# commanderson/morna

Measured on NVIDIA B200. Metric: exact kNN queries/s (50k samples x 3000 feats, k=100), higher is better.
Workload: dtype fp16 first pass (fp32 accumulate), f64 re-rank

## Files before the change

morna_b200/csrc/search_batched.cu:

```cuda
#include <cuda_fp16.h>
#include <limits.h>
#include <math.h>

#include "common.cuh"
#include "tc_ptx.cuh"

namespace morna {

constexpr int kPrepThreads = 256;

__global__ void __launch_bounds__(kPrepThreads)
prep_samples_kernel(const float *__restrict__ vectors, const double *__restrict__ pp, int64_t n, int64_t ld,
                    __half *__restrict__ hs, int64_t ld_h, float *__restrict__ rho_max) {
    const int lane = threadIdx.x & 31;
    const int64_t warps_total = (int64_t)gridDim.x * (kPrepThreads / 32);
    const int chunks = (int)(ld >> 2), chunks_h = (int)(ld_h >> 2);
    for (int64_t row = (int64_t)blockIdx.x * (kPrepThreads / 32) + (threadIdx.x >> 5); row < n; row += warps_total) {
        const float4 *src = reinterpret_cast<const float4 *>(vectors + row * ld);
        uint2 *dst = reinterpret_cast<uint2 *>(hs + row * ld_h);
        const double norm = sqrt(pp[row]);
        const double inv = norm > 0.0 ? 1.0 / norm : 0.0;
        double res = 0.0;
        for (int c = lane; c < chunks_h; c += 32) {
            float4 v = c < chunks ? ldg_stream_f4(src + c) : make_float4(0.f, 0.f, 0.f, 0.f);
// ... 637 lines not shown
                                if (j < valid) dst[j] = __uint_as_float(r[j]);
                        }
                    }
                } else {
                    uint32_t mask = 0;
#pragma unroll
                    for (int j = 0; j < 32; ++j)
                        mask |= (uint32_t)(__uint_as_float(r[j]) >= thr && j < valid) << j;
                    if (mask) {
                        int at = atomicAdd(p.cand_cnt + row, __popc(mask));
                        float *cs = p.cand_score + (int64_t)row * p.cap;
                        int32_t *ci = p.cand_id + (int64_t)row * p.cap;
#pragma unroll
                        for (int j = 0; j < 32; ++j) {
                            if ((mask >> j) & 1u) {
                                if (at < p.cap) { cs[at] = __uint_as_float(r[j]); ci[at] = p.id_base + col0 + j; }
                                ++at;
                            }
                        }
                    }
                }
            }
            tc_fence_before();
            mbar_arrive(tempty_bar(acc));
            if (++acc == ACC_STAGES) { acc = 0; acc_phase ^= 1; }
        }
    }
    tc_fence_before();
    __syncthreads();
    if (warp == 2) tmem_dealloc<1>(tmem_base, TMEM_COLS);
}

namespace gemm2 {
constexpr int BM = 128, BN = 256, BN_HALF = 128, BK = 64, UMMA_K = 16;
constexpr int A_BYTES = BM * BK * 2, B_BYTES = BN_HALF * BK * 2, STAGE_BYTES = A_BYTES + B_BYTES;
constexpr int THREADS = 192;
constexpr int HELPER_WARPS = 8;
constexpr int THREADS_ALL = THREADS + 32 * HELPER_WARPS;
constexpr int ACC_STAGES = 2, TMEM_COLS = ACC_STAGES * BN;
constexpr int HELPER_BYTES = HELPER_WARPS * 1024 * 4 + 16;
constexpr int smem_bytes(int stages) { return stages * STAGE_BYTES + 1024 + 256 + HELPER_BYTES; }
}

__device__ __forceinline__ uint32_t cluster_ctarank() {
    uint32_t r;
    asm volatile("mov.u32 %0, %%cluster_ctarank;" : "=r"(r));
    return r;
}
__device__ __forceinline__ void cluster_sync_all() {
    asm volatile("barrier.cluster.arrive.release.aligned;\n\tbarrier.cluster.wait.acquire.aligned;" ::: "memory");
}
__device__ __forceinline__ uint32_t mapa_rank(uint32_t addr, uint32_t rank) {
    uint32_t r;
    asm volatile("mapa.shared::cluster.u32 %0, %1, %2;" : "=r"(r) : "r"(addr), "r"(rank));
    return r;
}

template <int kStages, bool kHelpers, int kCluster>
__device__ __forceinline__ void
knn_gemm2_body(const CUtensorMap &tmap_q, const CUtensorMap &tmap_s, const GemmParams &p, const RerankParams &rr) {
    using namespace gemm2;
    constexpr bool kQuad = kCluster == 4;
    using namespace tc;
    extern __shared__ uint8_t smem_raw[];
    const uint32_t base = (smem_u32(smem_raw) + 1023u) & ~1023u;
    const uint32_t bars = base + kStages * STAGE_BYTES;
    auto full_bar = [&](int s) { return bars + 8u * s; };
    auto empty_bar = [&](int s) { return bars + 8u * (kStages + s); };
    auto tfull_bar = [&](int a) { return bars + 8u * (2 * kStages + a); };
    auto tempty_bar = [&](int a) { return bars + 8u * (2 * kStages + ACC_STAGES + a); };
    const uint32_t tmem_slot = bars + 8u * (2 * kStages + 2 * ACC_STAGES);
    volatile uint32_t *tmem_slot_ptr =
        reinterpret_cast<volatile uint32_t *>(smem_raw + (tmem_slot - smem_u32(smem_raw)));
    int *helper_lists = reinterpret_cast<int *>(smem_raw + (bars + 256u - smem_u32(smem_raw)));
    volatile int *helper_stop = helper_lists + (kHelpers ? HELPER_WARPS * 1024 : 0);

    const int warp = threadIdx.x >> 5, lane = threadIdx.x & 31;
    const uint32_t crank = cluster_ctarank();
    const uint32_t rank = crank & 1u;
    const uint32_t leader_rank = crank & ~1u;
    const int pair_in_cluster = (int)(crank >> 1);
    const bool leader = rank == 0;
    if (warp == 0 && lane == 0) {
        prefetch_tmap(&tmap_q);
        prefetch_tmap(&tmap_s);
    }
    if (warp == 1 && lane == 0) {
        for (int s = 0; s < kStages; ++s) { mbar_init(full_bar(s), 1); mbar_init(empty_bar(s), kQuad ? 2 : 1); }
        for (int a = 0; a < ACC_STAGES; ++a) { mbar_init(tfull_bar(a), 1); mbar_init(tempty_bar(a), 256); }
        fence_barrier_init();
        *helper_stop = 0;
    }
    if (warp == 2) {
        tmem_alloc<2>(tmem_slot, TMEM_COLS);
        tmem_relinquish<2>();
    }
    tc_fence_before();
    cluster_sync_all();
    tc_fence_after();
    const uint32_t tmem_base = *tmem_slot_ptr;

    const int pair = blockIdx.x / kCluster, pairs = gridDim.x / kCluster;
    const int m_pairs = (p.m_blocks + 1) >> 1;
    const int m_groups = kQuad ? (m_pairs + 1) >> 1 : m_pairs;
    const int total_tiles = m_groups * p.n_tiles;
    auto m_pair_of = [&](int t) { return kQuad ? 2 * (t % m_groups) + pair_in_cluster : t % m_groups; };
    if (warp == 0) {
        if (lane == 0) {
            int stage = 0; uint32_t phase = 0;
            uint64_t keep = 0;
            if (p.l2_keep) asm volatile("createpolicy.fractional.L2::evict_last.b64 %0, 1.0;" : "=l"(keep));
            for (int t = pair; t < total_tiles; t += pairs) {
                const int m_pair = m_pair_of(t), n_tile = t / m_groups;
                const int row_q = m_pair * 2 * BM + (int)rank * BM;
                const int row_s = p.n_begin + n_tile * BN + (int)rank * BN_HALF + (kQuad ? pair_in_cluster * (BN_HALF / 2) : 0);
                for (int kb = 0; kb < p.kblocks; ++kb) {
                    if (p.relaxed_ns > 1) mbar_wait_relaxed(empty_bar(stage), phase ^ 1, 20u);
                    else mbar_wait(empty_bar(stage), phase ^ 1);
                    const uint32_t a_dst = base + stage * STAGE_BYTES, b_dst = a_dst + A_BYTES;
                    const uint32_t bar0 = mapa_rank(full_bar(stage), leader_rank);
                    if (leader) mbar_expect_tx(full_bar(stage), 2 * STAGE_BYTES);
                    if (p.l2_keep) tma_load_2d_pair_hint(a_dst, &tmap_q, bar0, kb * BK, row_q, keep);
                    else tma_load_2d_pair(a_dst, &tmap_q, bar0, kb * BK, row_q);
                    if (kQuad)
                        tma_load_2d_pair_multicast(b_dst + pair_in_cluster * (B_BYTES / 2), &tmap_s, bar0, kb * BK, row_s,
                                                   (uint16_t)((1u << crank) | (1u << (crank ^ 2u))));
                    else if (p.l2_keep)
                        tma_load_2d_pair_hint(b_dst, &tmap_s, bar0, kb * BK, row_s, keep);
                    else
                        tma_load_2d_pair(b_dst, &tmap_s, bar0, kb * BK, row_s);
                    if (++stage == kStages) { stage = 0; phase ^= 1; }
                }
            }
        }
    } else if (warp == 1) {
        if (lane == 0 && leader) {
            constexpr uint32_t idesc = instr_desc_f16(2 * BM, BN,  0);
            int stage = 0; uint32_t phase = 0; int acc = 0; uint32_t acc_phase = 0;
            long long w_full = 0, w_acc = 0;
            const long long t_begin = clock64();
            for (int t = pair; t < total_tiles; t += pairs) {
                long long c0 = p.debug ? clock64() : 0;
                mbar_wait(tempty_bar(acc), acc_phase ^ 1);
                if (p.debug) w_acc += clock64() - c0;
                tc_fence_after();
                const uint32_t d_tmem = tmem_base + acc * BN;
                for (int kb = 0; kb < p.kblocks; ++kb) {
                    c0 = p.debug ? clock64() : 0;
                    mbar_wait(full_bar(stage), phase);
                    if (p.debug) w_full += clock64() - c0;
                    tc_fence_after();
                    const uint32_t a_src = base + stage * STAGE_BYTES, b_src = a_src + A_BYTES;
                    const uint64_t da = smem_desc_sw128(a_src), db = smem_desc_sw128(b_src);
#pragma unroll
                    for (int k = 0; k < BK / UMMA_K; ++k)
                        umma_f16<2>(d_tmem, da + 2 * k, db + 2 * k, idesc, (kb | k) != 0);
                    umma_commit_pair(empty_bar(stage), kQuad ? 0xF : 0x3);
                    if (kb == p.kblocks - 1) umma_commit_pair(tfull_bar(acc), (uint16_t)(0x3u << leader_rank));
                    if (++stage == kStages) { stage = 0; phase ^= 1; }
                }
                if (++acc == ACC_STAGES) { acc = 0; acc_phase ^= 1; }
            }
            if (p.debug) { p.debug[blockIdx.x * 4 + 0] = w_full; p.debug[blockIdx.x * 4 + 1] = w_acc; p.debug[blockIdx.x * 4 + 2] = clock64() - t_begin; }
        }
    } else if (kHelpers && warp >= THREADS / 32) {
        if (rr.queue) rerank_warp_loop<8, 2>(rr, helper_lists + (warp - THREADS / 32) * 1024, lane, helper_stop);
    } else {
        const int quarter = warp & 3;
        int acc = 0; uint32_t acc_phase = 0;
        long long e_busy = 0;
        for (int t = pair; t < total_tiles; t += pairs) {
            const int m_pair = m_pair_of(t), n_tile = t / m_groups;
            const int row = m_pair * 2 * BM + (int)rank * BM + quarter * 32 + lane;
            const bool row_ok = row < p.nq;
            const int col_tile = p.n_begin + n_tile * BN;
            float thr = INFINITY;
            if (p.mode == 1 && row_ok) thr = p.thr[row];
            if (p.relaxed_ns) mbar_wait_relaxed(tfull_bar(acc), acc_phase, (unsigned)p.relaxed_ns);
            else mbar_wait(tfull_bar(acc), acc_phase);
            const long long e0 = p.debug ? clock64() : 0;
            tc_fence_after();
            const uint32_t taddr = tmem_base + ((uint32_t)(quarter * 32) << 16) + acc * BN;
#pragma unroll 1
            for (int c = 0; c < BN / 32; ++c) {
                uint32_t r[32];
                tmem_ld_32x32(taddr + c * 32, r);
                tmem_ld_wait();
                const int col0 = col_tile + c * 32;
                const int valid = min(32, p.n_end - col0);
                if (p.mode == 0) {
                    if (row_ok && valid > 0) {
                        float *dst = p.pilot + (int64_t)row * p.pilot_ld + (col0 - p.n_begin);
                        if (valid == 32) {
#pragma unroll
                            for (int j = 0; j < 32; j += 4)
                                *reinterpret_cast<float4 *>(dst + j) =
                                    make_float4(__uint_as_float(r[j]), __uint_as_float(r[j + 1]),
                                                __uint_as_float(r[j + 2]), __uint_as_float(r[j + 3]));
                        } else {
#pragma unroll
                            for (int j = 0; j < 32; ++j)
                                if (j < valid) dst[j] = __uint_as_float(r[j]);
                        }
                    }
                } else {
                    uint32_t mask = 0;
#pragma unroll
                    for (int j = 0; j < 32; ++j)
                        mask |= (uint32_t)(__uint_as_float(r[j]) >= thr && j < valid) << j;
                    if (mask && !p.dry_epilogue) {
                        int at = atomicAdd(p.cand_cnt + row, __popc(mask));
                        float *cs = p.cand_score + (int64_t)row * p.cap;
                        int32_t *ci = p.cand_id + (int64_t)row * p.cap;
#pragma unroll
                        for (int j = 0; j < 32; ++j) {
                            if ((mask >> j) & 1u) {
                                if (at < p.cap) { cs[at] = __uint_as_float(r[j]); ci[at] = p.id_base + col0 + j; }
                                ++at;
                            }
                        }
                    }
                }
            }
            tc_fence_before();
            mbar_arrive_cluster(tempty_bar(acc), leader_rank);
            if (p.debug) e_busy += clock64() - e0;
            if (++acc == ACC_STAGES) { acc = 0; acc_phase ^= 1; }
        }
        if (p.debug && warp == 2 && lane == 0) p.debug[blockIdx.x * 4 + 3] = e_busy;
        if (warp == 2 && lane == 0) *helper_stop = 1;
    }
    tc_fence_before();
    cluster_sync_all();
    if (warp == 2) tmem_dealloc<2>(tmem_base, TMEM_COLS);
}

template <int kStages, bool kHelpers>
__global__ void __cluster_dims__(2, 1, 1) __launch_bounds__(kHelpers ? gemm2::THREADS_ALL : gemm2::THREADS, 1)
knn_gemm2_kernel(const __grid_constant__ CUtensorMap tmap_q, const __grid_constant__ CUtensorMap tmap_s, GemmParams p,
                 const RerankParams rr) {
    knn_gemm2_body<kStages, kHelpers, 2>(tmap_q, tmap_s, p, rr);
}

template <int kStages>
__global__ void __cluster_dims__(4, 1, 1) __launch_bounds__(gemm2::THREADS, 1)
knn_gemm4_kernel(const __grid_constant__ CUtensorMap tmap_q, const __grid_constant__ CUtensorMap tmap_s, GemmParams p,
                 const RerankParams rr) {
    knn_gemm2_body<kStages, false, 4>(tmap_q, tmap_s, p, rr);
}

constexpr int kKthThreads = 256, kKthItems = 32, kKthMax = kKthThreads * kKthItems;

__device__ __forceinline__ uint32_t float_key(float v) {
    uint32_t b = __float_as_uint(v);
    return (b & 0x80000000u) ? ~b : (b | 0x80000000u);
}
__device__ __forceinline__ float key_float(uint32_t k) {
    return __uint_as_float((k & 0x80000000u) ? (k & 0x7fffffffu) : ~k);
}

struct KthParams {
    int32_t k, n0, n_begin, id_base, cap, fcap;
    const float *pilot; int64_t pilot_ld;
    const float *eps;
    float *thr;
    float *cand_score; int32_t *cand_id; int32_t *cand_cnt;
    float *cand2_score; int32_t *cand2_id;
    int32_t *fin_id; int32_t *fin_cnt;
    uint8_t *overflow; int32_t *stats;
    float *kth_bound;
};

template <int kItems>
__device__ __forceinline__ uint32_t warp_kth_largest(const uint32_t (&key)[kItems], int kk) {
    uint32_t hi = 0u, lo = ~0u;
#pragma unroll
    for (int j = 0; j < kItems; ++j) { hi = max(hi, key[j]); lo = min(lo, key[j] ? key[j] : ~0u); }
    hi = __reduce_max_sync(kFull, hi);
    lo = __reduce_min_sync(kFull, lo);
    if (hi == 0u || kk <= 0) return 0u;
    const int first = 31 - __clz((int)(hi ^ lo) | 1);
// ... 283 lines not shown
    CUresult r = fn(map, CU_TENSOR_MAP_DATA_TYPE_FLOAT16, 2, const_cast<void *>(ptr), dims, strides, box, estr,
                    CU_TENSOR_MAP_INTERLEAVE_NONE, CU_TENSOR_MAP_SWIZZLE_128B, promo, CU_TENSOR_MAP_FLOAT_OOB_FILL_NONE);
    if (r != CUDA_SUCCESS) { g_last_cuda_error = (int)r; return MORNA_ERR_CUDA; }
    return MORNA_OK;
}

static int sm_count_b() { return sm_count_current(); }

constexpr int kCandCap = kCandCapConst, kFinCap = 1024, kPilotMax = kKthMax;
constexpr int64_t kBatchedMaxRows = (int64_t)1 << 24;

static int g_gemm_pair = 1;
static int g_gemm_stages = 4;
static int g_block_rows = 131072;
static int g_pilot_rows = kKthMax;
static int g_block_growth = 1;
static int g_first_block = 0;
static int g_rerank_ctas_per_sm = 0;
static int g_rerank_rows = 4;
static int g_rerank_phase_mb = -1;
static int g_rerank_kernel = 1;
static int g_rerank_ctas = 0;
static int g_rerank_subs = 0;
static int g_side_job = 0;
static int g_rerank_sort_rows = 1;
static int g_rerank_evict_first = 0;
static int g_gemm_l2_keep = 0;
static int g_rerank_fat_sms = 0;
static int g_gemm_pairs_cap = 0;
static int g_rerank_pipe = 1;
static long long *g_gemm_debug = nullptr;
static int g_gemm_relaxed_ns = 0;
static int g_gemm_dry = 0;
static int g_carveout_hint = 0;
static int g_rerank_oneshot = 1;


static int launch_knn_gemm(const CUtensorMap &tmap_q, const CUtensorMap &tmap_s, const GemmParams &gp, cudaStream_t s,
                           const RerankParams *side = nullptr) {
    if (!g_gemm_pair) {
        int rca = ensure_dynamic_smem((const void *)knn_gemm_kernel, gemm::SMEM_BYTES);
        if (rca != MORNA_OK) return rca;
        int tiles = gp.m_blocks * gp.n_tiles;
        int grid = tiles < sm_count_b() ? tiles : sm_count_b();
        knn_gemm_kernel<<<grid, gemm::THREADS, gemm::SMEM_BYTES, s>>>(tmap_q, tmap_s, gp);
        MORNA_LAUNCH_CHECK();
        return MORNA_OK;
    }
    if (g_gemm_pair == 2 && !side && (gp.m_blocks % 4) == 0) {
        auto kern4 = knn_gemm4_kernel<4>;
        const int smem4 = gemm2::smem_bytes(4) - gemm2::HELPER_BYTES + 16;
        int rca = ensure_dynamic_smem((const void *)kern4, smem4);
        if (rca != MORNA_OK) return rca;
        int tiles4 = (gp.m_blocks / 4) * gp.n_tiles;
        int clusters = 0;
        cudaLaunchConfig_t cfg{};
        cfg.gridDim = dim3(4 * (sm_count_b() / 4)); cfg.blockDim = dim3(gemm2::THREADS); cfg.dynamicSmemBytes = smem4; cfg.stream = s;
        if (cudaOccupancyMaxActiveClusters(&clusters, kern4, &cfg) != cudaSuccess || clusters < 1) { cudaGetLastError(); clusters = sm_count_b() / 4; }
        if (clusters > sm_count_b() / 4) clusters = sm_count_b() / 4;
        if (tiles4 < clusters) clusters = tiles4;
        RerankParams none{};
        kern4<<<4 * clusters, gemm2::THREADS, smem4, s>>>(tmap_q, tmap_s, gp, none);
        MORNA_LAUNCH_CHECK();
        return MORNA_OK;
    }
    const int stages = g_gemm_stages == 4 ? 4 : 6;
    auto kern = side ? (stages == 4 ? knn_gemm2_kernel<4, true> : knn_gemm2_kernel<6, true>)
                     : (stages == 4 ? knn_gemm2_kernel<4, false> : knn_gemm2_kernel<6, false>);
    const int smem = gemm2::smem_bytes(stages);
    int rca = ensure_dynamic_smem((const void *)kern, smem);
    if (rca != MORNA_OK) return rca;
    int tiles = ((gp.m_blocks + 1) / 2) * gp.n_tiles;
    int pairs = sm_count_b() / 2;
    if (g_gemm_pairs_cap > 0 && pairs > g_gemm_pairs_cap) pairs = g_gemm_pairs_cap;
    if (tiles < pairs) pairs = tiles;
    RerankParams rr{};
    if (side) rr = *side;
    if (g_carveout_hint) cudaFuncSetAttribute((const void *)kern, cudaFuncAttributePreferredSharedMemoryCarveout, cudaSharedmemCarveoutMaxShared);
    const int threads = side ? gemm2::THREADS_ALL : gemm2::THREADS;
    const int smem_launch = side ? smem : smem - gemm2::HELPER_BYTES + 16;
    kern<<<2 * pairs, threads, smem_launch, s>>>(tmap_q, tmap_s, gp, rr);
    MORNA_LAUNCH_CHECK();
    return MORNA_OK;
}

struct BatchWs {
    size_t hq, qq, eps, pilot, thr, cand_score, cand_id, cand2_score, cand2_id, cand_cnt, fin_id, fin_cnt, fin_dist, queue, total;
    int64_t nq_pad, n0, pilot_ld;
};
static BatchWs batch_ws_layout(int64_t n, int64_t nq, int64_t ld_h) {
    BatchWs w{};
    w.nq_pad = (nq + 2 * gemm::BM - 1) / (2 * gemm::BM) * (2 * gemm::BM);
    w.n0 = n < g_pilot_rows ? n : g_pilot_rows;
    if (w.n0 > g_block_rows) w.n0 = g_block_rows;
    w.pilot_ld = (w.n0 + 3) / 4 * 4;
    size_t off = 0;
    auto take = [&](size_t bytes) { size_t at = off; off += align_up(bytes, 256); return at; };
    w.hq = take((size_t)w.nq_pad * ld_h * sizeof(__half));
    w.qq = take((size_t)nq * sizeof(double));
    w.eps = take((size_t)nq * sizeof(float));
    w.pilot = take((size_t)nq * w.pilot_ld * sizeof(float));
    w.thr = take((size_t)nq * sizeof(float));
    w.cand_score = take((size_t)nq * kCandCap * sizeof(float));
    w.cand_id = take((size_t)nq * kCandCap * sizeof(int32_t));
    if (n > g_block_rows || (g_first_block > 0 && n > g_first_block)) {
        w.cand2_score = take((size_t)nq * kCandCap * sizeof(float));
        w.cand2_id = take((size_t)nq * kCandCap * sizeof(int32_t));
    }
    w.cand_cnt = take((size_t)nq * sizeof(int32_t));
    w.fin_id = take((size_t)nq * kFinCap * sizeof(int32_t));
    w.fin_cnt = take((size_t)nq * sizeof(int32_t));
    w.fin_dist = take((size_t)nq * kFinCap * sizeof(double));
    w.queue = take(sizeof(unsigned long long));
    w.total = off + 1024;
// ... 53 lines not shown
        if (rcj != MORNA_OK) return rcj;
        if (warp_kernel && side_jobs_enabled()) side_ptr = &side;
    }
    cudaStream_t s = (cudaStream_t)stream;
    unsigned char *ws = (unsigned char *)workspace;
    __half *hq = (__half *)(ws + w.hq);
    double *qq = (double *)(ws + w.qq);
    float *eps = (float *)(ws + w.eps);
    float *pilot = (float *)(ws + w.pilot);
    float *thr = (float *)(ws + w.thr);
    float *cand_score = (float *)(ws + w.cand_score);
    int32_t *cand_id = (int32_t *)(ws + w.cand_id);
    int32_t *cand_cnt = (int32_t *)(ws + w.cand_cnt);
    int32_t *fin_id = (int32_t *)(ws + w.fin_id);
    int32_t *fin_cnt = (int32_t *)(ws + w.fin_cnt);

    int phase = 0;
    auto mark = [&]() { if (phase_events) cudaEventRecord((cudaEvent_t)phase_events[phase], s); ++phase; };
    mark();
    MORNA_CUDA_TRY(cudaMemsetAsync(overflow, 0, (size_t)nq, s));
    MORNA_CUDA_TRY(cudaMemsetAsync(stats, 0, 4 * sizeof(int32_t), s));
    MORNA_CUDA_TRY(cudaMemsetAsync(cand_cnt, 0, (size_t)nq * sizeof(int32_t), s));
    MORNA_CUDA_TRY(cudaMemsetAsync(ws + w.queue, 0, sizeof(unsigned long long), s));

    const float eps_acc = (float)((double)(dim / 16 + 8) * 2.384185791015625e-07 * 1.01);
    {
        int64_t blocks = (w.nq_pad + 7) / 8;
        if (blocks > (int64_t)sm_count_b() * 8) blocks = (int64_t)sm_count_b() * 8;
        prep_queries_kernel<<<(unsigned)blocks, kPrepThreads, 0, s>>>(queries, nq, w.nq_pad, dim, q_ld, hq, ld_h, qq,
                                                                    eps, rho_max, eps_acc, overflow, stats);
        MORNA_LAUNCH_CHECK();
    }
    mark();
    CUtensorMap tmap_q, tmap_s;
    int rc = make_tmap(&tmap_q, hq, (uint64_t)w.nq_pad, (uint64_t)ld_h, gemm::BM);
    if (rc != MORNA_OK) return rc;
    rc = make_tmap(&tmap_s, hs, (uint64_t)n, (uint64_t)ld_h,
                   g_gemm_pair == 2 && !side_ptr && (w.nq_pad / gemm::BM) % 4 == 0 ? gemm2::BN_HALF / 2 : g_gemm_pair ? gemm2::BN_HALF : gemm::BN);
    if (rc != MORNA_OK) return rc;
    GemmParams gp{};
    gp.debug = g_gemm_debug; gp.relaxed_ns = g_gemm_relaxed_ns; gp.dry_epilogue = g_gemm_dry; gp.l2_keep = g_gemm_l2_keep;
    gp.nq = (int32_t)nq; gp.kblocks = (int32_t)(ld_h / gemm::BK); gp.m_blocks = (int32_t)(w.nq_pad / gemm::BM);
    gp.cap = kCandCap; gp.id_base = id_base; gp.pilot = pilot; gp.pilot_ld = w.pilot_ld; gp.thr = thr;
    gp.cand_score = cand_score; gp.cand_id = cand_id; gp.cand_cnt = cand_cnt;
    auto launch_gemm = [&](int32_t n_begin, int32_t n_end, int32_t mode) -> int {
        gp.n_begin = n_begin; gp.n_end = n_end; gp.mode = mode;
        gp.n_tiles = (n_end - n_begin + gemm::BN - 1) / gemm::BN;
        return launch_knn_gemm(tmap_q, tmap_s, gp, s, side_ptr);
    };
    KthParams kp{};
    kp.k = k; kp.n0 = (int32_t)w.n0; kp.n_begin = 0; kp.id_base = id_base; kp.cap = kCandCap; kp.fcap = kFinCap;
    kp.pilot = pilot; kp.pilot_ld = w.pilot_ld; kp.eps = eps; kp.thr = thr; kp.cand_score = cand_score;
    kp.cand_id = cand_id; kp.cand_cnt = cand_cnt; kp.fin_id = fin_id; kp.fin_cnt = fin_cnt; kp.overflow = overflow;
    kp.stats = stats;
    if ((rc = ensure_dynamic_smem((const void *)kth_warp_kernel<1>, kKwSmem)) != MORNA_OK) return rc;
    if ((rc = ensure_dynamic_smem((const void *)kth_warp_kernel<0>, kKwSmem)) != MORNA_OK) return rc;
    if ((rc = ensure_dynamic_smem((const void *)kth_warp_kernel<2>, kKwSmem)) != MORNA_OK) return rc;
    const unsigned kth_grid = (unsigned)((nq + kKwWarps - 1) / kKwWarps);

    rc = launch_gemm(0, (int32_t)w.n0, 0);
    if (rc != MORNA_OK) return rc;
    mark();
    kth_warp_kernel<1><<<kth_grid, kKwWarps * 32, kKwSmem, s>>>(kp, (int)nq);
    MORNA_LAUNCH_CHECK();
    mark();
    int64_t step = g_block_rows;
    for (int64_t b0 = w.n0; b0 < n;) {
        int64_t b1 = b0 == w.n0 ? (int64_t)(g_first_block > 0 ? g_first_block : g_block_rows) : b0 + step;
        if (b0 != w.n0 && g_block_growth > 1) step *= g_block_growth;
        if (b1 <= b0) b1 = b0 + step;
        if (b1 > n) b1 = n;
        rc = launch_gemm((int32_t)b0, (int32_t)b1, 1);
        if (rc != MORNA_OK) return rc;
        b0 = b1;
        if (b0 < n) {
            kp.cand2_score = (float *)(ws + w.cand2_score);
            kp.cand2_id = (int32_t *)(ws + w.cand2_id);
            kth_warp_kernel<2><<<kth_grid, kKwWarps * 32, kKwSmem, s>>>(kp, (int)nq);
            MORNA_LAUNCH_CHECK();
            float *ts = kp.cand_score; kp.cand_score = kp.cand2_score; kp.cand2_score = ts;
            int32_t *ti = kp.cand_id; kp.cand_id = kp.cand2_id; kp.cand2_id = ti;
// ... 287 lines not shown
extern "C" int morna_knn_batched(const float *vectors, const double *pp, const void *hs, int64_t ld_h,
                                 const float *rho_max, int64_t n, int32_t dim, int64_t ld, int32_t id_base,
                                 const double *queries, int64_t nq, int64_t q_ld, int32_t k, int32_t *out_ids,
                                 double *out_dist, uint8_t *overflow, int32_t *stats, void *workspace,
                                 size_t workspace_bytes, void *const *phase_events, void *stream) {
    if (!vectors || !pp || !out_ids || !out_dist || ld < dim || (ld & 3)) return MORNA_ERR_INVALID_ARGUMENT;
    int rc = morna_knn_batched_score(hs, ld_h, rho_max, n, dim, id_base, queries, nq, q_ld, k, overflow, stats,
                                     workspace, workspace_bytes, phase_events, nullptr, nullptr, stream);
    if (rc != MORNA_OK) return rc;
    rc = morna_knn_batched_rerank(vectors, pp, n, dim, ld, id_base, queries, nq, q_ld, k, out_ids, out_dist, overflow,
                                  workspace, workspace_bytes, 0, stream);
    if (rc == MORNA_OK && phase_events) cudaEventRecord((cudaEvent_t)phase_events[6], (cudaStream_t)stream);
    return rc;
}

extern "C" int morna_debug_tensor_scores(const void *hs, int64_t ld_h, const float *rho_max, int64_t n, int32_t dim,
                                         const double *queries, int64_t nq, int64_t q_ld, float *scores,
                                         int64_t scores_ld, float *eps_out, void *workspace, size_t workspace_bytes,
                                         void *stream) {
    if (!hs || !rho_max || !queries || !scores || !eps_out || n <= 0 || nq <= 0 || scores_ld < n || (scores_ld & 3) ||
        ld_h != morna_tensor_operand_ld(dim))
        return MORNA_ERR_INVALID_ARGUMENT;
    BatchWs w = batch_ws_layout(n, nq, ld_h);
    if (!workspace || workspace_bytes < w.total) return MORNA_ERR_WORKSPACE_TOO_SMALL;
    cudaStream_t s = (cudaStream_t)stream;
    unsigned char *ws = (unsigned char *)workspace;
    __half *hq = (__half *)(ws + w.hq);
    double *qq = (double *)(ws + w.qq);
    const float eps_acc = (float)((double)(dim / 16 + 8) * 2.384185791015625e-07 * 1.01);
    int64_t blocks = (w.nq_pad + 7) / 8;
    prep_queries_kernel<<<(unsigned)blocks, kPrepThreads, 0, s>>>(queries, nq, w.nq_pad, dim, q_ld, hq, ld_h, qq,
                                                                eps_out, rho_max, eps_acc, nullptr, nullptr);
    MORNA_LAUNCH_CHECK();
    CUtensorMap tmap_q, tmap_s;
    int rc = make_tmap(&tmap_q, hq, (uint64_t)w.nq_pad, (uint64_t)ld_h, gemm::BM);
    if (rc != MORNA_OK) return rc;
    rc = make_tmap(&tmap_s, hs, (uint64_t)n, (uint64_t)ld_h,
                   g_gemm_pair == 2 && (w.nq_pad / gemm::BM) % 4 == 0 ? gemm2::BN_HALF / 2 : g_gemm_pair ? gemm2::BN_HALF : gemm::BN);
    if (rc != MORNA_OK) return rc;
    GemmParams gp{};
    gp.nq = (int32_t)nq; gp.kblocks = (int32_t)(ld_h / gemm::BK); gp.m_blocks = (int32_t)(w.nq_pad / gemm::BM);
    gp.n_begin = 0; gp.n_end = (int32_t)n; gp.mode = 0; gp.pilot = scores; gp.pilot_ld = scores_ld;
    gp.n_tiles = (gp.n_end + gemm::BN - 1) / gemm::BN;
    return launch_knn_gemm(tmap_q, tmap_s, gp, s);
}

namespace morna {

constexpr int kRangeMaxQueries = 4096;
constexpr int kRangeWarps = 8;
constexpr int kRangeEmitThreads = 512;

struct RangeWs {
    size_t hq, qq, eps, thr, cand_score, cand_id, cand_cnt, match_id, match_dist, match_cnt, prep_stats, total;
    int64_t nq_pad;
};
static RangeWs range_ws_layout(int64_t nq, int64_t ld_h) {
    RangeWs w{};
    w.nq_pad = (nq + 2 * gemm::BM - 1) / (2 * gemm::BM) * (2 * gemm::BM);
    size_t off = 0;
    auto take = [&](size_t bytes) { size_t at = off; off += align_up(bytes, 256); return at; };
    w.hq = take((size_t)w.nq_pad * ld_h * sizeof(__half));
    w.qq = take((size_t)nq * sizeof(double));
    w.eps = take((size_t)nq * sizeof(float));
    w.thr = take((size_t)nq * sizeof(float));
    w.cand_score = take((size_t)nq * kCandCap * sizeof(float));
    w.cand_id = take((size_t)nq * kCandCap * sizeof(int32_t));
    w.cand_cnt = take((size_t)nq * sizeof(int32_t));
    w.match_id = take((size_t)nq * kCandCap * sizeof(int32_t));
    w.match_dist = take((size_t)nq * kCandCap * sizeof(double));
    w.match_cnt = take((size_t)nq * sizeof(int32_t));
    w.prep_stats = take(4 * sizeof(int32_t));
    w.total = off + 1024;
    return w;
}

__global__ void range_thr_kernel(const float *__restrict__ eps, const uint8_t *__restrict__ overflow, int32_t nq, double R,
// ... 128 lines not shown
                                   int64_t q_ld, double max_distance, int32_t *counts, uint8_t *overflow, int64_t *stats,
                                   void *workspace, size_t workspace_bytes, void *stream) {
    if (!vectors || !pp || !hs || !rho_max || !queries || !counts || !overflow || !stats || n <= 0 || n > kBatchedMaxRows ||
        nq <= 0 || nq > kRangeMaxQueries || dim <= 0 || ld < dim || (ld & 3) || q_ld < dim ||
        ld_h != morna_tensor_operand_ld(dim) || !(max_distance >= 0.0) || isinf(max_distance))
        return MORNA_ERR_INVALID_ARGUMENT;
    const RangeWs w = range_ws_layout(nq, ld_h);
    if (!workspace || workspace_bytes < w.total) return MORNA_ERR_WORKSPACE_TOO_SMALL;
    cudaStream_t s = (cudaStream_t)stream;
    unsigned char *ws = (unsigned char *)workspace;
    __half *hq = (__half *)(ws + w.hq);
    double *qq = (double *)(ws + w.qq);
    float *eps = (float *)(ws + w.eps);
    float *thr = (float *)(ws + w.thr);
    int32_t *cand_cnt = (int32_t *)(ws + w.cand_cnt);
    int32_t *match_cnt = (int32_t *)(ws + w.match_cnt);
    MORNA_CUDA_TRY(cudaMemsetAsync(overflow, 0, (size_t)nq, s));
    MORNA_CUDA_TRY(cudaMemsetAsync(stats, 0, 4 * sizeof(int64_t), s));
    MORNA_CUDA_TRY(cudaMemsetAsync(cand_cnt, 0, (size_t)nq * sizeof(int32_t), s));
    MORNA_CUDA_TRY(cudaMemsetAsync(match_cnt, 0, (size_t)nq * sizeof(int32_t), s));
    MORNA_CUDA_TRY(cudaMemsetAsync(ws + w.prep_stats, 0, 4 * sizeof(int32_t), s));

    const float eps_acc = (float)((double)(dim / 16 + 8) * 2.384185791015625e-07 * 1.01);
    {
        int64_t blocks = (w.nq_pad + 7) / 8;
        if (blocks > (int64_t)sm_count_b() * 8) blocks = (int64_t)sm_count_b() * 8;
        prep_queries_kernel<<<(unsigned)blocks, kPrepThreads, 0, s>>>(queries, nq, w.nq_pad, dim, q_ld, hq, ld_h, qq, eps, rho_max,
                                                                    eps_acc, overflow, (int32_t *)(ws + w.prep_stats));
        MORNA_LAUNCH_CHECK();
    }
    range_thr_kernel<<<(unsigned)((nq + 255) / 256), 256, 0, s>>>(eps, overflow, (int32_t)nq, max_distance, thr);
    MORNA_LAUNCH_CHECK();

    CUtensorMap tmap_q, tmap_s;
    int rc = make_tmap(&tmap_q, hq, (uint64_t)w.nq_pad, (uint64_t)ld_h, gemm::BM);
    if (rc != MORNA_OK) return rc;
    rc = make_tmap(&tmap_s, hs, (uint64_t)n, (uint64_t)ld_h,
                   g_gemm_pair == 2 && (w.nq_pad / gemm::BM) % 4 == 0 ? gemm2::BN_HALF / 2 : g_gemm_pair ? gemm2::BN_HALF : gemm::BN);
    if (rc != MORNA_OK) return rc;
    GemmParams gp{};
    gp.debug = g_gemm_debug; gp.relaxed_ns = g_gemm_relaxed_ns; gp.l2_keep = g_gemm_l2_keep;
    gp.nq = (int32_t)nq; gp.kblocks = (int32_t)(ld_h / gemm::BK); gp.m_blocks = (int32_t)(w.nq_pad / gemm::BM);
    gp.cap = kCandCap; gp.id_base = id_base; gp.thr = thr;
    gp.cand_score = (float *)(ws + w.cand_score); gp.cand_id = (int32_t *)(ws + w.cand_id); gp.cand_cnt = cand_cnt;
    gp.n_begin = 0; gp.n_end = (int32_t)n; gp.mode = 1;
    gp.n_tiles = (int32_t)((n + gemm::BN - 1) / gemm::BN);
    if ((rc = launch_knn_gemm(tmap_q, tmap_s, gp, s)) != MORNA_OK) return rc;

    RangeCheckParams cp{};
    cp.vectors = vectors; cp.pp = pp; cp.ld = ld; cp.dim = dim; cp.id_base = id_base; cp.nq = (int32_t)nq;
    cp.queries = queries; cp.q_ld = q_ld; cp.qq = qq; cp.cand_id = gp.cand_id; cp.cand_cnt = cand_cnt; cp.overflow = overflow;
    cp.R = max_distance; cp.match_id = (int32_t *)(ws + w.match_id); cp.match_dist = (double *)(ws + w.match_dist);
    cp.match_cnt = match_cnt;
    int per_sm = 0;
    MORNA_CUDA_TRY(cudaOccupancyMaxActiveBlocksPerMultiprocessor(&per_sm, range_check_kernel, kRangeWarps * 32, 0));
    if (per_sm < 1) per_sm = 1;
    const int64_t items = nq * (kCandCap / 32);
    int64_t grid = (int64_t)per_sm * sm_count_b();
    if (grid * kRangeWarps > items) grid = (items + kRangeWarps - 1) / kRangeWarps;
    range_check_kernel<<<(unsigned)grid, kRangeWarps * 32, 0, s>>>(cp);
    MORNA_LAUNCH_CHECK();
    range_finish_kernel<<<(unsigned)((nq + 255) / 256), 256, 0, s>>>(cand_cnt, match_cnt, (int32_t)nq, overflow, counts,
                                                                    (unsigned long long *)stats);
    MORNA_LAUNCH_CHECK();
    return MORNA_OK;
}

extern "C" int morna_range_batched_emit(int64_t n, int64_t nq, int32_t dim, const int64_t *offsets, const uint8_t *overflow,
                                        int32_t *out_ids, double *out_dist, const void *workspace, size_t workspace_bytes,
                                        void *stream) {
    if (!offsets || !overflow || !out_ids || !out_dist || n <= 0 || n > kBatchedMaxRows || nq <= 0 || nq > kRangeMaxQueries ||
        dim <= 0)
        return MORNA_ERR_INVALID_ARGUMENT;
    const RangeWs w = range_ws_layout(nq, morna_tensor_operand_ld(dim));
    if (!workspace || workspace_bytes < w.total) return MORNA_ERR_WORKSPACE_TOO_SMALL;
    const unsigned char *ws = (const unsigned char *)workspace;
    const size_t smem = (size_t)kCandCap * (sizeof(double) + sizeof(int));
    { int rca = ensure_dynamic_smem((const void *)range_emit_kernel, smem); if (rca != MORNA_OK) return rca; }
    range_emit_kernel<<<(unsigned)nq, kRangeEmitThreads, smem, (cudaStream_t)stream>>>(
        (const int32_t *)(ws + w.match_id), (const double *)(ws + w.match_dist), (const int32_t *)(ws + w.match_cnt), overflow,
// ... 11 lines not shown
    else if (key == 3) morna::set_single_tma(value);
    else if (key == 4) morna::set_acc_pipelined(value);
    else if (key == 1) g_gemm_stages = value;
    else if (key == 5) g_rerank_rows = value;
    else if (key == 13) g_rerank_ctas_per_sm = value;
    else if (key == 9) g_block_rows = value >= 256 ? value : 131072;
    else if (key == 10) g_pilot_rows = value >= 256 && value <= kPilotMax ? value : kPilotMax;
    else if (key == 11) g_first_block = value > 0 ? value : 0;
    else if (key == 7) morna::set_acc_split(value);
    else if (key == 8) morna::set_acc_variant(value);
    else if (key == 12) morna::set_acc_shift(value);
    else if (key == 25) morna::set_ids_early_exit(value);
    else if (key == 27) morna::set_single_prefetch(value);
    else if (key == 28) morna::set_single_prefetch_rows(value);
    else if (key == 29) morna::set_single_chain(value);
    else if (key == 35) morna::set_sparse_tile_mb(value);
    else if (key == 36) g_block_growth = value >= 1 && value <= 8 ? value : 1;
    else if (key == 6) g_rerank_phase_mb = value;
    else if (key == 14) g_rerank_kernel = value;
    else if (key == 15) g_rerank_ctas = value;
    else if (key == 16) g_rerank_subs = value;
    else if (key == 17) g_side_job = value;
    else if (key == 18) g_rerank_pipe = value;
    else if (key == 32) g_rerank_evict_first = value >= 0 && value <= 4 ? value : 0;
    else if (key == 33) g_gemm_l2_keep = value ? 1 : 0;
    else if (key == 34) g_rerank_sort_rows = value ? 1 : 0;
    else if (key == 30) g_rerank_fat_sms = value > 0 ? value : 0;
    else if (key == 31) g_gemm_pairs_cap = value > 0 ? value : 0;
    else if (key == 19) g_carveout_hint = value;
    else if (key == 20) g_rerank_oneshot = value;
    else if (key == 22) g_gemm_relaxed_ns = value;
    else if (key == 23) g_gemm_dry = value;
    else if (key == 24) g_tmap_promotion = value;

    else return MORNA_ERR_INVALID_ARGUMENT;
    return MORNA_OK;
}
```

Before: 2.222 million.

## Add 512-wide pair GEMM tile with staged candidate epilogue and double-buffered TMEM loads

Adds a 512-column variant of the 2-CTA pair GEMM. It issues two 256-wide UMMAs per k-step, uses a single TMEM accumulator, and runs eight epilogue warps. The wide tile is picked automatically when it does not raise per-pair tile-wave count, aiming to reuse each query tile across more sample columns. The epilogue now double-buffers TMEM loads, releases the accumulator earlier, and stages candidates in shared memory to cut global atomics per row. The trade-off is losing accumulator double-buffering and using fewer pipeline stages in wide mode, and sample tensor maps are now rebuilt on every launch.

```diff
diff --git a/morna_b200/csrc/search_batched.cu b/morna_b200/csrc/search_batched.cu
--- a/morna_b200/csrc/search_batched.cu
+++ b/morna_b200/csrc/search_batched.cu
@@ -693,14 +693,24 @@
 }
 
 namespace gemm2 {
-constexpr int BM = 128, BN = 256, BN_HALF = 128, BK = 64, UMMA_K = 16;
-constexpr int A_BYTES = BM * BK * 2, B_BYTES = BN_HALF * BK * 2, STAGE_BYTES = A_BYTES + B_BYTES;
+constexpr int BM = 128, BN_HALF = 128, BK = 64, UMMA_K = 16, UMMA_N = 256;
+constexpr int A_BYTES = BM * BK * 2, B_HALF_BYTES = BN_HALF * BK * 2;
 constexpr int THREADS = 192;
 constexpr int HELPER_WARPS = 8;
 constexpr int THREADS_ALL = THREADS + 32 * HELPER_WARPS;
-constexpr int ACC_STAGES = 2, TMEM_COLS = ACC_STAGES * BN;
+constexpr int TMEM_COLS = 512;
 constexpr int HELPER_BYTES = HELPER_WARPS * 1024 * 4 + 16;
-constexpr int smem_bytes(int stages) { return stages * STAGE_BYTES + 1024 + 256 + HELPER_BYTES; }
+constexpr int STAGE_SLOTS = 16;
+constexpr int epi_warps(int bn) { return bn / 64; }
+constexpr int threads(int bn) { return 64 + 32 * epi_warps(bn); }
+constexpr int stage_bytes(int bn) { return A_BYTES + (bn / UMMA_N) * B_HALF_BYTES; }
+constexpr int slots(bool helpers) { return helpers ? 0 : STAGE_SLOTS; }
+constexpr int staging_bytes(int bn, bool helpers) { return epi_warps(bn) * 32 * slots(helpers) * 8; }
+constexpr int smem_bytes(int stages, int bn, bool helpers) {
+    return stages * stage_bytes(bn) + 1024 + 256 + staging_bytes(bn, helpers) + (helpers ? HELPER_BYTES : 16);
+}
+static_assert(smem_bytes(6, 256, true) <= 227 * 1024 && smem_bytes(6, 256, false) <= 227 * 1024 &&
+              smem_bytes(4, 512, false) <= 227 * 1024, "shared memory budget");
 }
 
 __device__ __forceinline__ uint32_t cluster_ctarank() {
@@ -717,23 +727,29 @@
     return r;
 }
 
-template <int kStages, bool kHelpers, int kCluster>
+template <int kStages, bool kHelpers, int kCluster, int kBN>
 __device__ __forceinline__ void
 knn_gemm2_body(const CUtensorMap &tmap_q, const CUtensorMap &tmap_s, const GemmParams &p, const RerankParams &rr) {
     using namespace gemm2;
+    static_assert(kBN == 256 || (kBN == 512 && !kHelpers && kCluster == 2), "the 512-wide tile is a plain pair kernel");
     constexpr bool kQuad = kCluster == 4;
+    constexpr int kAcc = TMEM_COLS / kBN;
+    constexpr int kStageBytes = stage_bytes(kBN);
+    constexpr int kEpiWarps = epi_warps(kBN), kSlots = slots(kHelpers);
+    constexpr int kNmma = kBN / UMMA_N;
     using namespace tc;
     extern __shared__ uint8_t smem_raw[];
     const uint32_t base = (smem_u32(smem_raw) + 1023u) & ~1023u;
-    const uint32_t bars = base + kStages * STAGE_BYTES;
+    const uint32_t bars = base + kStages * kStageBytes;
     auto full_bar = [&](int s) { return bars + 8u * s; };
     auto empty_bar = [&](int s) { return bars + 8u * (kStages + s); };
     auto tfull_bar = [&](int a) { return bars + 8u * (2 * kStages + a); };
-    auto tempty_bar = [&](int a) { return bars + 8u * (2 * kStages + ACC_STAGES + a); };
-    const uint32_t tmem_slot = bars + 8u * (2 * kStages + 2 * ACC_STAGES);
+    auto tempty_bar = [&](int a) { return bars + 8u * (2 * kStages + kAcc + a); };
+    const uint32_t tmem_slot = bars + 8u * (2 * kStages + 2 * kAcc);
     volatile uint32_t *tmem_slot_ptr =
         reinterpret_cast<volatile uint32_t *>(smem_raw + (tmem_slot - smem_u32(smem_raw)));
-    int *helper_lists = reinterpret_cast<int *>(smem_raw + (bars + 256u - smem_u32(smem_raw)));
+    uint2 *staging = reinterpret_cast<uint2 *>(smem_raw + (bars + 256u - smem_u32(smem_raw)));
+    int *helper_lists = reinterpret_cast<int *>(staging + kEpiWarps * kSlots * 32);
     volatile int *helper_stop = helper_lists + (kHelpers ? HELPER_WARPS * 1024 : 0);
 
     const int warp = threadIdx.x >> 5, lane = threadIdx.x & 31;
@@ -748,7 +764,7 @@
     }
     if (warp == 1 && lane == 0) {
         for (int s = 0; s < kStages; ++s) { mbar_init(full_bar(s), 1); mbar_init(empty_bar(s), kQuad ? 2 : 1); }
-        for (int a = 0; a < ACC_STAGES; ++a) { mbar_init(tfull_bar(a), 1); mbar_init(tempty_bar(a), 256); }
+        for (int a = 0; a < kAcc; ++a) { mbar_init(tfull_bar(a), 1); mbar_init(tempty_bar(a), 2 * 32 * kEpiWarps); }
         fence_barrier_init();
         *helper_stop = 0;
     }
@@ -774,29 +790,33 @@
             for (int t = pair; t < total_tiles; t += pairs) {
                 const int m_pair = m_pair_of(t), n_tile = t / m_groups;
                 const int row_q = m_pair * 2 * BM + (int)rank * BM;
-                const int row_s = p.n_begin + n_tile * BN + (int)rank * BN_HALF + (kQuad ? pair_in_cluster * (BN_HALF / 2) : 0);
+                const int row_s = p.n_begin + n_tile * kBN + (int)rank * BN_HALF + (kQuad ? pair_in_cluster * (BN_HALF / 2) : 0);
                 for (int kb = 0; kb < p.kblocks; ++kb) {
                     if (p.relaxed_ns > 1) mbar_wait_relaxed(empty_bar(stage), phase ^ 1, 20u);
                     else mbar_wait(empty_bar(stage), phase ^ 1);
-                    const uint32_t a_dst = base + stage * STAGE_BYTES, b_dst = a_dst + A_BYTES;
+                    const uint32_t a_dst = base + stage * kStageBytes, b_dst = a_dst + A_BYTES;
                     const uint32_t bar0 = mapa_rank(full_bar(stage), leader_rank);
-                    if (leader) mbar_expect_tx(full_bar(stage), 2 * STAGE_BYTES);
+                    if (leader) mbar_expect_tx(full_bar(stage), 2 * kStageBytes);
                     if (p.l2_keep) tma_load_2d_pair_hint(a_dst, &tmap_q, bar0, kb * BK, row_q, keep);
                     else tma_load_2d_pair(a_dst, &tmap_q, bar0, kb * BK, row_q);
-                    if (kQuad)
-                        tma_load_2d_pair_multicast(b_dst + pair_in_cluster * (B_BYTES / 2), &tmap_s, bar0, kb * BK, row_s,
-                                                   (uint16_t)((1u << crank) | (1u << (crank ^ 2u))));
-                    else if (p.l2_keep)
-                        tma_load_2d_pair_hint(b_dst, &tmap_s, bar0, kb * BK, row_s, keep);
-                    else
-                        tma_load_2d_pair(b_dst, &tmap_s, bar0, kb * BK, row_s);
+#pragma unroll
+                    for (int j = 0; j < kNmma; ++j) {
+                        const uint32_t dst = b_dst + j * B_HALF_BYTES;
+                        if (kQuad)
+                            tma_load_2d_pair_multicast(dst + pair_in_cluster * (B_HALF_BYTES / 2), &tmap_s, bar0, kb * BK, row_s,
+                                                       (uint16_t)((1u << crank) | (1u << (crank ^ 2u))));
+                        else if (p.l2_keep)
+                            tma_load_2d_pair_hint(dst, &tmap_s, bar0, kb * BK, row_s + j * UMMA_N, keep);
+                        else
+                            tma_load_2d_pair(dst, &tmap_s, bar0, kb * BK, row_s + j * UMMA_N);
+                    }
                     if (++stage == kStages) { stage = 0; phase ^= 1; }
                 }
             }
         }
     } else if (warp == 1) {
         if (lane == 0 && leader) {
-            constexpr uint32_t idesc = instr_desc_f16(2 * BM, BN,  0);
+            constexpr uint32_t idesc = instr_desc_f16(2 * BM, UMMA_N,  0);
             int stage = 0; uint32_t phase = 0; int acc = 0; uint32_t acc_phase = 0;
             long long w_full = 0, w_acc = 0;
             const long long t_begin = clock64();
@@ -805,22 +825,25 @@
                 mbar_wait(tempty_bar(acc), acc_phase ^ 1);
                 if (p.debug) w_acc += clock64() - c0;
                 tc_fence_after();
-                const uint32_t d_tmem = tmem_base + acc * BN;
+                const uint32_t d_tmem = tmem_base + acc * kBN;
                 for (int kb = 0; kb < p.kblocks; ++kb) {
                     c0 = p.debug ? clock64() : 0;
                     mbar_wait(full_bar(stage), phase);
                     if (p.debug) w_full += clock64() - c0;
                     tc_fence_after();
-                    const uint32_t a_src = base + stage * STAGE_BYTES, b_src = a_src + A_BYTES;
-                    const uint64_t da = smem_desc_sw128(a_src), db = smem_desc_sw128(b_src);
+                    const uint32_t a_src = base + stage * kStageBytes, b_src = a_src + A_BYTES;
+                    const uint64_t da = smem_desc_sw128(a_src);
 #pragma unroll
                     for (int k = 0; k < BK / UMMA_K; ++k)
-                        umma_f16<2>(d_tmem, da + 2 * k, db + 2 * k, idesc, (kb | k) != 0);
+#pragma unroll
+                        for (int j = 0; j < kNmma; ++j)
+                            umma_f16<2>(d_tmem + j * UMMA_N, da + 2 * k, smem_desc_sw128(b_src + j * B_HALF_BYTES) + 2 * k, idesc,
+                                        (kb | k) != 0);
                     umma_commit_pair(empty_bar(stage), kQuad ? 0xF : 0x3);
                     if (kb == p.kblocks - 1) umma_commit_pair(tfull_bar(acc), (uint16_t)(0x3u << leader_rank));
                     if (++stage == kStages) { stage = 0; phase ^= 1; }
                 }
-                if (++acc == ACC_STAGES) { acc = 0; acc_phase ^= 1; }
+                if (++acc == kAcc) { acc = 0; acc_phase ^= 1; }
             }
             if (p.debug) { p.debug[blockIdx.x * 4 + 0] = w_full; p.debug[blockIdx.x * 4 + 1] = w_acc; p.debug[blockIdx.x * 4 + 2] = clock64() - t_begin; }
         }
@@ -828,25 +851,24 @@
         if (rr.queue) rerank_warp_loop<8, 2>(rr, helper_lists + (warp - THREADS / 32) * 1024, lane, helper_stop);
     } else {
         const int quarter = warp & 3;
+        const int half = (warp - 2) / 4;
+        uint2 *slot = staging + (warp - 2) * kSlots * 32 + lane;
         int acc = 0; uint32_t acc_phase = 0;
         long long e_busy = 0;
         for (int t = pair; t < total_tiles; t += pairs) {
             const int m_pair = m_pair_of(t), n_tile = t / m_groups;
             const int row = m_pair * 2 * BM + (int)rank * BM + quarter * 32 + lane;
             const bool row_ok = row < p.nq;
-            const int col_tile = p.n_begin + n_tile * BN;
+            const int col_tile = p.n_begin + n_tile * kBN + half * UMMA_N;
             float thr = INFINITY;
             if (p.mode == 1 && row_ok) thr = p.thr[row];
             if (p.relaxed_ns) mbar_wait_relaxed(tfull_bar(acc), acc_phase, (unsigned)p.relaxed_ns);
             else mbar_wait(tfull_bar(acc), acc_phase);
             const long long e0 = p.debug ? clock64() : 0;
             tc_fence_after();
-            const uint32_t taddr = tmem_base + ((uint32_t)(quarter * 32) << 16) + acc * BN;
-#pragma unroll 1
-            for (int c = 0; c < BN / 32; ++c) {
-                uint32_t r[32];
-                tmem_ld_32x32(taddr + c * 32, r);
-                tmem_ld_wait();
+            const uint32_t taddr = tmem_base + ((uint32_t)(quarter * 32) << 16) + acc * kBN + half * UMMA_N;
+            int staged = 0;
+            auto chunk = [&](const uint32_t (&r)[32], int c) {
                 const int col0 = col_tile + c * 32;
                 const int valid = min(32, p.n_end - col0);
                 if (p.mode == 0) {
@@ -864,29 +886,59 @@
                                 if (j < valid) dst[j] = __uint_as_float(r[j]);
                         }
                     }
+                    return;
+                }
+                uint32_t mask = 0;
+#pragma unroll
+                for (int j = 0; j < 32; ++j)
+                    mask |= (uint32_t)(__uint_as_float(r[j]) >= thr && j < valid) << j;
+                if (!mask || p.dry_epilogue) return;
+                const int cnt = __popc(mask);
+                if (staged + cnt <= kSlots) {
+#pragma unroll
+                    for (int j = 0; j < 32; ++j)
+                        if ((mask >> j) & 1u) slot[32 * staged++] = make_uint2(r[j], (uint32_t)(p.id_base + col0 + j));
+                    return;
+                }
+                int at = atomicAdd(p.cand_cnt + row, cnt);
+                float *cs = p.cand_score + (int64_t)row * p.cap;
+                int32_t *ci = p.cand_id + (int64_t)row * p.cap;
+#pragma unroll
+                for (int j = 0; j < 32; ++j) {
+                    if ((mask >> j) & 1u) {
+                        if (at < p.cap) { cs[at] = __uint_as_float(r[j]); ci[at] = p.id_base + col0 + j; }
+                        ++at;
+                    }
+                }
+            };
+            uint32_t ra[32], rb[32];
+            tmem_ld_32x32(taddr, ra);
+#pragma unroll 1
+            for (int c = 0; c < UMMA_N / 32; c += 2) {
+                tmem_ld_wait();
+                tmem_ld_32x32(taddr + (c + 1) * 32, rb);
+                chunk(ra, c);
+                tmem_ld_wait();
+                if (c + 2 < UMMA_N / 32) {
+                    tmem_ld_32x32(taddr + (c + 2) * 32, ra);
                 } else {
-                    uint32_t mask = 0;
-#pragma unroll
-                    for (int j = 0; j < 32; ++j)
-                        mask |= (uint32_t)(__uint_as_float(r[j]) >= thr && j < valid) << j;
-                    if (mask && !p.dry_epilogue) {
-                        int at = atomicAdd(p.cand_cnt + row, __popc(mask));
-                        float *cs = p.cand_score + (int64_t)row * p.cap;
-                        int32_t *ci = p.cand_id + (int64_t)row * p.cap;
-#pragma unroll
-                        for (int j = 0; j < 32; ++j) {
-                            if ((mask >> j) & 1u) {
-                                if (at < p.cap) { cs[at] = __uint_as_float(r[j]); ci[at] = p.id_base + col0 + j; }
-                                ++at;
-                            }
-                        }
-                    }
-                }
-            }
-            tc_fence_before();
-            mbar_arrive_cluster(tempty_bar(acc), leader_rank);
+                    tc_fence_before();
+                    mbar_arrive_cluster(tempty_bar(acc), leader_rank);
+                }
+                chunk(rb, c + 1);
+            }
+            if (staged) {
+                int at = atomicAdd(p.cand_cnt + row, staged);
+                float *cs = p.cand_score + (int64_t)row * p.cap;
+                int32_t *ci = p.cand_id + (int64_t)row * p.cap;
+                for (int i = 0; i < staged && at < p.cap; ++i, ++at) {
+                    const uint2 e = slot[32 * i];
+                    cs[at] = __uint_as_float(e.x);
+                    ci[at] = (int32_t)e.y;
+                }
+            }
             if (p.debug) e_busy += clock64() - e0;
-            if (++acc == ACC_STAGES) { acc = 0; acc_phase ^= 1; }
+            if (++acc == kAcc) { acc = 0; acc_phase ^= 1; }
         }
         if (p.debug && warp == 2 && lane == 0) p.debug[blockIdx.x * 4 + 3] = e_busy;
         if (warp == 2 && lane == 0) *helper_stop = 1;
@@ -896,18 +948,18 @@
     if (warp == 2) tmem_dealloc<2>(tmem_base, TMEM_COLS);
 }
 
-template <int kStages, bool kHelpers>
-__global__ void __cluster_dims__(2, 1, 1) __launch_bounds__(kHelpers ? gemm2::THREADS_ALL : gemm2::THREADS, 1)
+template <int kStages, bool kHelpers, int kBN>
+__global__ void __cluster_dims__(2, 1, 1) __launch_bounds__(kHelpers ? gemm2::THREADS_ALL : gemm2::threads(kBN), 1)
 knn_gemm2_kernel(const __grid_constant__ CUtensorMap tmap_q, const __grid_constant__ CUtensorMap tmap_s, GemmParams p,
                  const RerankParams rr) {
-    knn_gemm2_body<kStages, kHelpers, 2>(tmap_q, tmap_s, p, rr);
+    knn_gemm2_body<kStages, kHelpers, 2, kBN>(tmap_q, tmap_s, p, rr);
 }
 
 template <int kStages>
 __global__ void __cluster_dims__(4, 1, 1) __launch_bounds__(gemm2::THREADS, 1)
 knn_gemm4_kernel(const __grid_constant__ CUtensorMap tmap_q, const __grid_constant__ CUtensorMap tmap_s, GemmParams p,
                  const RerankParams rr) {
-    knn_gemm2_body<kStages, false, 4>(tmap_q, tmap_s, p, rr);
+    knn_gemm2_body<kStages, false, 4, 256>(tmap_q, tmap_s, p, rr);
 }
 
 constexpr int kKthThreads = 256, kKthItems = 32, kKthMax = kKthThreads * kKthItems;
@@ -1257,15 +1309,21 @@
 static long long *g_gemm_debug = nullptr;
 static int g_gemm_relaxed_ns = 0;
 static int g_gemm_dry = 0;
+static int g_gemm_width = 0;
 static int g_carveout_hint = 0;
 static int g_rerank_oneshot = 1;
 
 
-static int launch_knn_gemm(const CUtensorMap &tmap_q, const CUtensorMap &tmap_s, const GemmParams &gp, cudaStream_t s,
+static int launch_knn_gemm(const CUtensorMap &tmap_q, const void *hs, int64_t n, int64_t ld_h, GemmParams gp, cudaStream_t s,
                            const RerankParams *side = nullptr) {
+    CUtensorMap tmap_s;
+    const int rows = gp.n_end - gp.n_begin;
     if (!g_gemm_pair) {
-        int rca = ensure_dynamic_smem((const void *)knn_gemm_kernel, gemm::SMEM_BYTES);
-        if (rca != MORNA_OK) return rca;
+        gp.n_tiles = (rows + gemm::BN - 1) / gemm::BN;
+        int rc = make_tmap(&tmap_s, hs, (uint64_t)n, (uint64_t)ld_h, gemm::BN);
+        if (rc != MORNA_OK) return rc;
+        rc = ensure_dynamic_smem((const void *)knn_gemm_kernel, gemm::SMEM_BYTES);
+        if (rc != MORNA_OK) return rc;
         int tiles = gp.m_blocks * gp.n_tiles;
         int grid = tiles < sm_count_b() ? tiles : sm_count_b();
         knn_gemm_kernel<<<grid, gemm::THREADS, gemm::SMEM_BYTES, s>>>(tmap_q, tmap_s, gp);
@@ -1273,10 +1331,13 @@
         return MORNA_OK;
     }
     if (g_gemm_pair == 2 && !side && (gp.m_blocks % 4) == 0) {
+        gp.n_tiles = (rows + 255) / 256;
+        int rc = make_tmap(&tmap_s, hs, (uint64_t)n, (uint64_t)ld_h, gemm2::BN_HALF / 2);
+        if (rc != MORNA_OK) return rc;
         auto kern4 = knn_gemm4_kernel<4>;
-        const int smem4 = gemm2::smem_bytes(4) - gemm2::HELPER_BYTES + 16;
-        int rca = ensure_dynamic_smem((const void *)kern4, smem4);
-        if (rca != MORNA_OK) return rca;
+        const int smem4 = gemm2::smem_bytes(4, 256, false);
+        rc = ensure_dynamic_smem((const void *)kern4, smem4);
+        if (rc != MORNA_OK) return rc;
         int tiles4 = (gp.m_blocks / 4) * gp.n_tiles;
         int clusters = 0;
         cudaLaunchConfig_t cfg{};
@@ -1289,22 +1350,35 @@
         MORNA_LAUNCH_CHECK();
         return MORNA_OK;
     }
-    const int stages = g_gemm_stages == 4 ? 4 : 6;
-    auto kern = side ? (stages == 4 ? knn_gemm2_kernel<4, true> : knn_gemm2_kernel<6, true>)
-                     : (stages == 4 ? knn_gemm2_kernel<4, false> : knn_gemm2_kernel<6, false>);
-    const int smem = gemm2::smem_bytes(stages);
-    int rca = ensure_dynamic_smem((const void *)kern, smem);
-    if (rca != MORNA_OK) return rca;
-    int tiles = ((gp.m_blocks + 1) / 2) * gp.n_tiles;
     int pairs = sm_count_b() / 2;
     if (g_gemm_pairs_cap > 0 && pairs > g_gemm_pairs_cap) pairs = g_gemm_pairs_cap;
-    if (tiles < pairs) pairs = tiles;
+    const int m_pairs = (gp.m_blocks + 1) / 2;
+    const int64_t narrow = (int64_t)m_pairs * ((rows + 255) / 256), wide = (int64_t)m_pairs * ((rows + 511) / 512);
+    const bool wide_ok = !side && g_gemm_width != 1;
+    const bool use_wide = wide_ok && (g_gemm_width == 2 || 2 * ((wide + pairs - 1) / pairs) <= (narrow + pairs - 1) / pairs);
+    const int bn = use_wide ? 512 : 256;
+    gp.n_tiles = (rows + bn - 1) / bn;
+    int rc = make_tmap(&tmap_s, hs, (uint64_t)n, (uint64_t)ld_h, gemm2::BN_HALF);
+    if (rc != MORNA_OK) return rc;
+    int stages;
+    auto kern = knn_gemm2_kernel<4, false, 256>;
+    if (use_wide) {
+        stages = g_gemm_stages == 3 ? 3 : 4;
+        kern = stages == 3 ? knn_gemm2_kernel<3, false, 512> : knn_gemm2_kernel<4, false, 512>;
+    } else {
+        stages = g_gemm_stages == 4 ? 4 : 6;
+        kern = side ? (stages == 4 ? knn_gemm2_kernel<4, true, 256> : knn_gemm2_kernel<6, true, 256>)
+                    : (stages == 4 ? knn_gemm2_kernel<4, false, 256> : knn_gemm2_kernel<6, false, 256>);
+    }
+    const int smem = gemm2::smem_bytes(stages, bn, side != nullptr);
+    const int threads = side ? gemm2::THREADS_ALL : gemm2::threads(bn);
+    if ((rc = ensure_dynamic_smem((const void *)kern, smem)) != MORNA_OK) return rc;
+    const int64_t tiles = use_wide ? wide : narrow;
+    if (tiles < pairs) pairs = (int)tiles;
     RerankParams rr{};
     if (side) rr = *side;
     if (g_carveout_hint) cudaFuncSetAttribute((const void *)kern, cudaFuncAttributePreferredSharedMemoryCarveout, cudaSharedmemCarveoutMaxShared);
-    const int threads = side ? gemm2::THREADS_ALL : gemm2::THREADS;
-    const int smem_launch = side ? smem : smem - gemm2::HELPER_BYTES + 16;
-    kern<<<2 * pairs, threads, smem_launch, s>>>(tmap_q, tmap_s, gp, rr);
+    kern<<<2 * pairs, threads, smem, s>>>(tmap_q, tmap_s, gp, rr);
     MORNA_LAUNCH_CHECK();
     return MORNA_OK;
 }
@@ -1424,11 +1498,8 @@
         MORNA_LAUNCH_CHECK();
     }
     mark();
-    CUtensorMap tmap_q, tmap_s;
+    CUtensorMap tmap_q;
     int rc = make_tmap(&tmap_q, hq, (uint64_t)w.nq_pad, (uint64_t)ld_h, gemm::BM);
-    if (rc != MORNA_OK) return rc;
-    rc = make_tmap(&tmap_s, hs, (uint64_t)n, (uint64_t)ld_h,
-                   g_gemm_pair == 2 && !side_ptr && (w.nq_pad / gemm::BM) % 4 == 0 ? gemm2::BN_HALF / 2 : g_gemm_pair ? gemm2::BN_HALF : gemm::BN);
     if (rc != MORNA_OK) return rc;
     GemmParams gp{};
     gp.debug = g_gemm_debug; gp.relaxed_ns = g_gemm_relaxed_ns; gp.dry_epilogue = g_gemm_dry; gp.l2_keep = g_gemm_l2_keep;
@@ -1437,8 +1508,7 @@
     gp.cand_score = cand_score; gp.cand_id = cand_id; gp.cand_cnt = cand_cnt;
     auto launch_gemm = [&](int32_t n_begin, int32_t n_end, int32_t mode) -> int {
         gp.n_begin = n_begin; gp.n_end = n_end; gp.mode = mode;
-        gp.n_tiles = (n_end - n_begin + gemm::BN - 1) / gemm::BN;
-        return launch_knn_gemm(tmap_q, tmap_s, gp, s, side_ptr);
+        return launch_knn_gemm(tmap_q, hs, n, ld_h, gp, s, side_ptr);
     };
     KthParams kp{};
     kp.k = k; kp.n0 = (int32_t)w.n0; kp.n_begin = 0; kp.id_base = id_base; kp.cap = kCandCap; kp.fcap = kFinCap;
@@ -1792,17 +1862,13 @@
     prep_queries_kernel<<<(unsigned)blocks, kPrepThreads, 0, s>>>(queries, nq, w.nq_pad, dim, q_ld, hq, ld_h, qq,
                                                                 eps_out, rho_max, eps_acc, nullptr, nullptr);
     MORNA_LAUNCH_CHECK();
-    CUtensorMap tmap_q, tmap_s;
+    CUtensorMap tmap_q;
     int rc = make_tmap(&tmap_q, hq, (uint64_t)w.nq_pad, (uint64_t)ld_h, gemm::BM);
-    if (rc != MORNA_OK) return rc;
-    rc = make_tmap(&tmap_s, hs, (uint64_t)n, (uint64_t)ld_h,
-                   g_gemm_pair == 2 && (w.nq_pad / gemm::BM) % 4 == 0 ? gemm2::BN_HALF / 2 : g_gemm_pair ? gemm2::BN_HALF : gemm::BN);
     if (rc != MORNA_OK) return rc;
     GemmParams gp{};
     gp.nq = (int32_t)nq; gp.kblocks = (int32_t)(ld_h / gemm::BK); gp.m_blocks = (int32_t)(w.nq_pad / gemm::BM);
     gp.n_begin = 0; gp.n_end = (int32_t)n; gp.mode = 0; gp.pilot = scores; gp.pilot_ld = scores_ld;
-    gp.n_tiles = (gp.n_end + gemm::BN - 1) / gemm::BN;
-    return launch_knn_gemm(tmap_q, tmap_s, gp, s);
+    return launch_knn_gemm(tmap_q, hs, n, ld_h, gp, s);
 }
 
 namespace morna {
@@ -1997,11 +2063,8 @@
     range_thr_kernel<<<(unsigned)((nq + 255) / 256), 256, 0, s>>>(eps, overflow, (int32_t)nq, max_distance, thr);
     MORNA_LAUNCH_CHECK();
 
-    CUtensorMap tmap_q, tmap_s;
+    CUtensorMap tmap_q;
     int rc = make_tmap(&tmap_q, hq, (uint64_t)w.nq_pad, (uint64_t)ld_h, gemm::BM);
-    if (rc != MORNA_OK) return rc;
-    rc = make_tmap(&tmap_s, hs, (uint64_t)n, (uint64_t)ld_h,
-                   g_gemm_pair == 2 && (w.nq_pad / gemm::BM) % 4 == 0 ? gemm2::BN_HALF / 2 : g_gemm_pair ? gemm2::BN_HALF : gemm::BN);
     if (rc != MORNA_OK) return rc;
     GemmParams gp{};
     gp.debug = g_gemm_debug; gp.relaxed_ns = g_gemm_relaxed_ns; gp.l2_keep = g_gemm_l2_keep;
@@ -2009,8 +2072,7 @@
     gp.cap = kCandCap; gp.id_base = id_base; gp.thr = thr;
     gp.cand_score = (float *)(ws + w.cand_score); gp.cand_id = (int32_t *)(ws + w.cand_id); gp.cand_cnt = cand_cnt;
     gp.n_begin = 0; gp.n_end = (int32_t)n; gp.mode = 1;
-    gp.n_tiles = (int32_t)((n + gemm::BN - 1) / gemm::BN);
-    if ((rc = launch_knn_gemm(tmap_q, tmap_s, gp, s)) != MORNA_OK) return rc;
+    if ((rc = launch_knn_gemm(tmap_q, hs, n, ld_h, gp, s)) != MORNA_OK) return rc;
 
     RangeCheckParams cp{};
     cp.vectors = vectors; cp.pp = pp; cp.ld = ld; cp.dim = dim; cp.id_base = id_base; cp.nq = (int32_t)nq;
@@ -2088,6 +2150,7 @@
     else if (key == 22) g_gemm_relaxed_ns = value;
     else if (key == 23) g_gemm_dry = value;
     else if (key == 24) g_tmap_promotion = value;
+    else if (key == 37) g_gemm_width = value == 1 || value == 2 ? value : 0;
 
     else return MORNA_ERR_INVALID_ARGUMENT;
     return MORNA_OK;
```

Result: faster. 2.281 million (median of 6 runs) (+2.6%).
